# luisdamiano/sparseRGPs

Hardware: AMD Instinct MI355X
Metric: sparse-GP objective+gradient evals/sec at n=1e6, m=1024, d=8 (higher is better)
Workload: dtype f64; 1 GPU; C3: Titsias VI ELBO + gradient, n=1000000, m=1024, d=8, ard, P=10, knots fixed; n=1000000, m=1024, d=8, kernel=ard, parallelism=single

## Files before the change

include/sgp_diag.h:

```cpp
#ifndef SGP_DIAG_H
#define SGP_DIAG_H

#include <stdint.h>

#ifdef __cplusplus
extern "C" {
#endif

int sgp_diag_gj_pair(int device, int64_t m, const double* A, const double* B, double beta,
                     int per_step, double* invA, double* invS, double* logdet);

int sgp_diag_store_bw(int device, int64_t bytes, int reps, int pattern, double* gbs);

int sgp_diag_syrk_plan(int64_t n, int64_t m, int* plan, int* workgroups, double* t_balanced,
                       double* t_packed);

#ifdef __cplusplus
}
#endif
#endif
```

sparsergps_amd/_lib.py:

```python
from __future__ import annotations

import ctypes as C
import os
import threading

from ._build import LIB, VARIANT_ROOT, HipccMissing, build

_lock = threading.Lock()
_lib = None

c_double_p = C.POINTER(C.c_double)
c_int_p = C.POINTER(C.c_int)

SGP_OK, SGP_EINVAL, SGP_ENOTPD, SGP_EHIP, SGP_ENOMEM = 0, 1, 2, 3, 4
KERNELS = {"sqexp": 0, "ard": 1, "exp": 2}
SGP_FLAG_R_DET = 1
SGP_FLAG_OBJ_ONLY = 2
SGP_PRED_VI, SGP_PRED_LAPLACE, SGP_PRED_FULL, SGP_PRED_LAPLACE_FULL = 0, 1, 2, 3
SGP_EXPO_ROWS = 0.0
FAMILIES = {"poisson": 0, "bernoulli": 1}

PROTOTYPES = {
    "sgp_last_error": (C.c_char_p, []),
    "sgp_abi_version": (C.c_int, []),
# ... 24 lines not shown
                                C.c_double, C.c_uint, c_double_p, c_double_p]),
    "sgp_vi_red1_count": (C.c_int64, [C.c_int64]),
    "sgp_vi_red1_packed_count": (C.c_int64, [C.c_int64]),
    "sgp_ctx_set_packed_reduction": (C.c_int, [C.c_void_p, C.c_int]),
    "sgp_vi_red2_count": (C.c_int64, [C.c_int, C.c_int]),
    "sgp_vi_phase1": (C.c_int, [C.c_void_p, C.c_int, c_double_p, c_double_p, C.c_int64, C.c_int64,
                                C.c_double, C.c_void_p]),
    "sgp_vi_phase2": (C.c_int, [C.c_void_p, C.c_void_p, C.c_int64, C.c_uint, C.c_void_p]),
    "sgp_vi_finish": (C.c_int, [C.c_void_p, C.c_void_p, c_double_p, c_double_p]),
    "sgp_fitc_red1_count": (C.c_int64, [C.c_int64]),
    "sgp_fitc_red2_count": (C.c_int64, [C.c_int, C.c_int, C.c_int64]),
    "sgp_fitc_phase1": (C.c_int, [C.c_void_p, C.c_int, c_double_p, c_double_p, C.c_int64, C.c_int64,
                                  C.c_double, C.c_void_p]),
    "sgp_fitc_phase2": (C.c_int, [C.c_void_p, C.c_void_p, C.c_int64, C.c_uint, C.c_void_p]),
    "sgp_fitc_finish": (C.c_int, [C.c_void_p, C.c_void_p, c_double_p, c_double_p]),
    "sgp_lap_set_f": (C.c_int, [C.c_void_p, c_double_p, C.c_double]),
    "sgp_lap_set_expo": (C.c_int, [C.c_void_p, c_double_p, C.c_double]),
    "sgp_lap_set_family": (C.c_int, [C.c_void_p, C.c_int]),
    "sgp_diag_gj_pair": (C.c_int, [C.c_int, C.c_int64, c_double_p, c_double_p, C.c_double, C.c_int,
                                   c_double_p, c_double_p, c_double_p]),
    "sgp_diag_store_bw": (C.c_int, [C.c_int, C.c_int64, C.c_int, C.c_int, c_double_p]),
    "sgp_diag_syrk_plan": (C.c_int, [C.c_int64, C.c_int64, c_int_p, c_int_p, c_double_p,
                                     c_double_p]),
    "sgp_lap_get_f": (C.c_int, [C.c_void_p, c_double_p]),
    "sgp_lap_get_grad_psi": (C.c_int, [C.c_void_p, c_double_p]),
    "sgp_lap_objective_values": (C.c_int, [C.c_void_p, c_double_p, C.c_int, c_int_p]),
    "sgp_eval_laplace": (C.c_int, [C.c_void_p, C.c_int, c_double_p, c_double_p, C.c_int64,
                                   C.c_int64, C.c_double, C.c_double, C.c_double, C.c_int,
                                   c_double_p, c_double_p, c_int_p]),
    "sgp_lap_red_count": (C.c_int64, [C.c_int, C.c_int, C.c_int64]),
    "sgp_lap_begin": (C.c_int, [C.c_void_p, C.c_int, c_double_p, c_double_p, C.c_int64, C.c_int64,
                                C.c_double, C.c_double, C.c_double, C.c_int, C.c_uint,
                                C.c_void_p, C.POINTER(C.c_int64)]),
    "sgp_lap_step": (C.c_int, [C.c_void_p, C.c_void_p, C.c_void_p, C.POINTER(C.c_int64), c_int_p,
                               c_double_p, c_double_p, c_int_p]),
    "sgp_lap_nr": (C.c_int, [C.c_void_p, C.c_int, c_double_p, c_double_p, C.c_int64, C.c_int64,
                             C.c_double, C.c_double, C.c_double, C.c_int, c_double_p, c_int_p]),
    "sgp_eval_full": (C.c_int, [C.c_void_p, C.c_int, c_double_p, C.c_double, C.c_uint,
                                c_double_p, c_double_p]),
    "sgp_eval_full_laplace": (C.c_int, [C.c_void_p, C.c_int, c_double_p, C.c_double, C.c_double,
                                        C.c_double, C.c_int, C.c_uint, c_double_p, c_double_p,
                                        c_int_p]),
    "sgp_full_laplace_state": (C.c_int, [C.c_void_p, c_double_p, c_double_p]),
    "sgp_posterior_u": (C.c_int, [C.c_void_p, c_double_p, c_double_p, c_double_p]),
    "sgp_predict": (C.c_int, [C.c_int, C.c_int, c_double_p, C.c_double, C.c_int, C.c_int, c_double_p,
                              C.c_int64, C.c_int64, c_double_p, c_double_p, c_double_p, C.c_int64,
# ... 90 lines not shown
```

sparsergps_amd/csrc/capi.hip:

```cpp
#include <math.h>

#include <cmath>
#include <stdarg.h>
#include <stdio.h>
#include <stdlib.h>
#include <string.h>
#include <time.h>

#include <algorithm>
#include <string>
#include <vector>

#include "../../include/sgp.h"
#include "../../include/sgp_diag.h"
#include "sgp_internal.h"

#ifdef SGP_HOST_PROBE
extern "C" __attribute__((visibility("default"))) double sgp_probe_t[4] = {0.0, 0.0, 0.0, 0.0};
#endif
#include "sgp_probe.h"
#include "sgp_multi.h"

namespace {

// ... 170 lines not shown
  double* r = nullptr;
  double* K = nullptr;
  double* alpha = nullptr;
  double* zinv = nullptr;
  double* omega = nullptr;
  double* pvec = nullptr;
  double* rowq = nullptr;
  double* red2f = nullptr;
  double* U = nullptr;
  double *K22 = nullptr, *K22inv = nullptr, *Bm = nullptr, *Binv = nullptr, *Pm = nullptr;
  double *Xt = nullptr, *T1 = nullptr, *M3 = nullptr;
  double *Xt22 = nullptr, *T22 = nullptr;
  unsigned* gjs = nullptr;
  double *dinv = nullptr, *dinv22 = nullptr, *logd22 = nullptr, *logdB = nullptr;
  double *uvec = nullptr, *cdiag = nullptr;
  int* status = nullptr;
  double *red1 = nullptr, *red2 = nullptr;
  double *slab_syrk = nullptr, *slab_con = nullptr, *slab_small = nullptr, *sc = nullptr;
  double* sk_ws = nullptr;
  unsigned* sk_flags = nullptr;
  unsigned sk_epoch = 0;
  int sk_slots = 0;
  double* tslab = nullptr;
  double *tq = nullptr, *tp = nullptr;
  int tstore_state = 0;
  int64_t slab_syrk_cap = 0, slab_con_cap = 0, slab_small_cap = 0;
  KernParams kp;
  int64_t m = 0, mp = 0, n_global = 0;
  double delta = 0.0;
  unsigned flags = 0;
  bool knot_on = false;
  double *knot_slab = nullptr, *knot_part = nullptr, *knot_kmm = nullptr;
  std::vector<double> knot_raw;
  std::vector<double> hU;
  double* pin = nullptr;
  hipEvent_t ev_pin = nullptr;
  bool knots_valid = false;
  int64_t knots_mp = 0;
  uint64_t* khash = nullptr;
  int* kidx = nullptr;
  uint8_t* cflag = nullptr;
  int64_t knots_gen = 0;
  int64_t cflag_gen = -1;
  std::vector<double> xmin, xmax;
  int phase = 0;
  int last_mode = 0;
// ... 193 lines not shown
    } else {
      (void)hipGetLastError();
      if (c->tq) (void)hipFree(c->tq);
      if (c->tp) (void)hipFree(c->tp);
      c->tq = c->tp = nullptr;
      c->tstore_state = -1;
    }
  }
  return c->tstore_state == 1;
}

static bool fuse_tt(sgp_ctx* c) { return c->kp.d <= 8 && tstore_ready(c); }

void ctx_free(sgp_ctx* c) {
  void* ptrs[] = {c->X,      c->r,     c->K,      c->alpha,   c->zinv,  c->U,    c->K22,
                  c->K22inv, c->Bm,    c->Binv,   c->Pm,      c->Xt,    c->T1,   c->M3,
                  c->dinv,   c->logd22, c->logdB, c->uvec,    c->cdiag, c->status, c->red1,
                  c->red2,   c->slab_syrk, c->slab_con, c->slab_small, c->slab_aux, c->sc,
                  c->sk_ws,  c->sk_flags,
                  c->Xt22,   c->T22,    c->dinv22, c->omega, c->pvec, c->rowq, c->red2f,
                  c->y,      c->mu,     c->lv,     c->lm,    c->lslab, c->lred[0], c->lred[1],
                  c->Cprev,  c->lapAZ,  c->lapAB,  c->laprv,  c->fl,
                  c->knot_slab, c->knot_part, c->knot_kmm, c->tslab, c->tq, c->tp,
                  c->rr_dev, c->Sfull, c->gjs, c->mmpart, c->rsync};
  for (void* p : ptrs)
    if (p) hipFree(p);
  if (c->khash) hipFree(c->khash);
  if (c->kidx) hipFree(c->kidx);
  if (c->cflag) hipFree(c->cflag);
  if (c->ev_knots) hipEventDestroy(c->ev_knots);
  if (c->ev_pin) hipEventDestroy(c->ev_pin);
  if (c->pin) hipHostFree(c->pin);
  if (c->ev_k22) hipEventDestroy(c->ev_k22);
  if (c->ev_k22m) hipEventDestroy(c->ev_k22m);
  if (c->ev_s) hipEventDestroy(c->ev_s);
  if (c->ev_m3) hipEventDestroy(c->ev_m3);
  if (c->ev_bm) hipEventDestroy(c->ev_bm);
  if (c->ev_lo) hipEventDestroy(c->ev_lo);
  if (c->ev_t) hipEventDestroy(c->ev_t);
  if (c->aux && !c->borrowed_streams) hipStreamDestroy(c->aux);
  if (c->aux_lo && !c->borrowed_streams) hipStreamDestroy(c->aux_lo);
  for (hipEvent_t e : c->pool) hipEventDestroy(e);
  if (c->own && !c->borrowed_streams) hipStreamDestroy(c->own);
}

hipError_t upload_rows(double* dst, const double* src, int64_t n, int64_t n_pad) {
  std::vector<double> h((size_t)n_pad, 0.0);
// ... 337 lines not shown
  if (con_sk_enabled()) {
    int cus = 0;
    if (!st && hipDeviceGetAttribute(&cus, hipDeviceAttributeMultiprocessorCount, device) ==
                   hipSuccess && cus > 0)
      c->sk_slots = 2 * cus;
    if (c->sk_slots > 0) {
      st = st ? st : dalloc(&c->sk_ws, sgp_con_sk_doubles(c->sk_slots));
      st = st ? st : dalloc(&c->sk_flags, c->sk_slots + 1);
      if (!st && hipMemset(c->sk_flags, 0, sizeof(unsigned) * (c->sk_slots + 1)) != hipSuccess) {
        set_err("hipMemset of the contraction hand-over flags failed");
        st = SGP_EHIP;
      }
    }
  }
  c->slab_small_cap = std::max<int64_t>(SLAB_SMALL, mp * (SGP_MAXD + 2));
  st = st ? st : dalloc(&c->slab_small, c->slab_small_cap);
  st = st ? st : dalloc(&c->slab_aux, c->slab_small_cap);
  st = st ? st : dalloc(&c->rr_dev, 1);
  st = st ? st : dalloc(&c->mmpart, 3 * mp);
  st = st ? st : dalloc(&c->sc, SC_N);
  st = st ? st : dalloc(&c->y, np_);
  st = st ? st : dalloc(&c->mu, np_);
  st = st ? st : dalloc(&c->tslab, (np_ / 64) * mp);
  st = st ? st : dalloc(&c->khash, mp);
  st = st ? st : dalloc(&c->kidx, mp);
  st = st ? st : dalloc(&c->cflag, np_);
  if (!st && (hipHostMalloc(reinterpret_cast<void**>(&c->pin),
                            sizeof(double) * (mp * d + m_max + (m_max + 1) / 2 + 8 + RB_N),
                            hipHostMallocDefault) != hipSuccess ||
              hipEventCreateWithFlags(&c->ev_pin, hipEventDisableTiming) != hipSuccess)) {
    set_err("pinned staging allocation failed");
    st = SGP_ENOMEM;
  }
  if (st) {
    ctx_free(c);
    delete c;
    return st;
  }
  c->xmin.assign((size_t)d, 0.0);
  c->xmax.assign((size_t)d, 0.0);
  for (int q = 0; q < d; ++q) {
    double lo = X[q * ldx], hi = X[q * ldx];
    for (int64_t i = 1; i < n; ++i) {
      const double v = X[i + q * ldx];
      lo = v < lo ? v : lo;
      hi = v > hi ? v : hi;
// ... 358 lines not shown
    Scope t(c, "build_knm");
    if (SGP_VI_BUILD_NO_T)
      HIPCHK(launch_build_knm(kp, c->X, c->n_pad, c->n, c->n_pad, c->U, mpv, m, mpv, c->K,
                              c->stream, false));
    else
      HIPCHK(launch_build_knm_t(kp, c->X, c->n_pad, c->n, c->n_pad, c->U, mpv, m, mpv, c->K,
                                c->r, c->tslab, &t_rows, c->stream, false));
  }
  st = k22_sync(c);
  if (st) return st;
  {
    Scope t(c, "syrk");
    HIPCHK(launch_syrk_aug(c->K, c->n_pad, mpv, c->r, nullptr, c->slab_syrk, c->slab_syrk_cap,
                           red1, c->stream, 1, nullptr, 0));
  }
  HIPCHK(hipMemsetAsync(c->status, 0, sizeof(int) * 4, c->aux));
  HIPCHK(hipMemsetAsync(c->sc, 0, sizeof(double) * SC_N, c->aux));
  st = k22_build(c, kp.tau2);
  if (st) return st;
  const int64_t toff = vi_red1_toff(c, mpv);
  if (small_syrk && c->fused_vi) {
    c->t_deferred = true;
    c->t_rows_def = t_rows;
  } else if (small_syrk) {
    HIPCHK(launch_knot_reduce(c->tslab, t_rows, mpv, 1, c->T1, c->mp_max * c->mp_max,
                              red1 + toff, false, c->stream));
  } else {
    HIPCHK(hipStreamWaitEvent(c->aux_lo, c->ev_knots, 0));
    HIPCHK(hipMemsetAsync(red1, 0, sizeof(double) * (toff + mpv + 8), c->aux_lo));
    HIPCHK(launch_knot_reduce(c->tslab, t_rows, mpv, 1, c->T1, c->mp_max * c->mp_max,
                              red1 + toff, false, c->aux_lo));
    HIPCHK(hipStreamWaitEvent(c->aux_lo, c->ev_k22m, 0));
    HIPCHK(hipEventRecord(c->ev_lo, c->aux_lo));
    HIPCHK(hipStreamWaitEvent(c->stream, c->ev_lo, 0));
  }
  {
    Scope t(c, "syrk_reduce");
    HIPCHK(launch_syrk_aug(c->K, c->n_pad, mpv, c->r, nullptr, c->slab_syrk, c->slab_syrk_cap,
                           red1, c->stream, 2, nullptr, 0, c->rr_dev, c->pack_red1, false,
                           c->rsync));
  }
  const bool k22_after_syrk = (double)c->n_pad * (double)mpv * (double)mpv > 3e10;
  st = k22_factor(c, k22_after_syrk);
  if (st) return st;
  c->phase = 1;
  return SGP_OK;
}

static int k22_factor_launches(sgp_ctx* c, hipStream_t s) {
  const int64_t mp = c->mp;
  HIPCHK(dense_spd_inverse(c->K22inv, mp, c->Xt22, c->dinv22, c->logd22, c->status,
                           c->gjs + SGP_GJ_SYNC_WORDS, s));
  HIPCHK(launch_sum_and_diag(c->logd22, mp / SGP_DB, c->sc + SC_LD22, c->K22inv, mp, mp,
                             c->cdiag, s));
  return SGP_OK;
}

static int k22_sync(sgp_ctx* c) {
// ... 103 lines not shown
    HIPCHK(hipEventRecord(c->ev_bm, c->stream));
  }
  {
    HIPCHK(hipStreamWaitEvent(c->aux_lo, c->ev_bm, 0));
    HIPCHK(launch_vi_mm_scalars(t, c->uvec, c->mmpart, mp, red1 + toff + mp, c->sc + SC_TU,
                                c->sc + SC_TRBS, c->sc + SC_RR, c->aux_lo));
    HIPCHK(launch_sum_small(c->logdB, mp / SGP_DB, c->sc + SC_LDB, c->aux_lo));
    Scope tm(c, "contract_kmm", c->aux_lo);
    int nb = 0;
    HIPCHK(launch_contract_kmm(kp, c->U, c->mp, c->m, mp, c->uvec, c->K22inv, c->Binv, c->M3,
                               -0.5, 0.5, -1.0 / (2.0 * kp.tau2), nullptr, nullptr, 0.0,
                               c->slab_aux, c->slab_small_cap, &nb, c->aux_lo));
    HIPCHK(launch_colsum(c->slab_aux, nb, kp.P, c->sc + SC_G22, c->aux_lo));
  }
  int st2 = SGP_OK;
  {
    Scope tm(c, "contract_knm");
    ConArgs ca;
    ca.r = c->r;
    ca.invz = 1.0 / z;
    ca.uvec = c->uvec;
    ca.cdiag = c->cdiag;
    ca.vi_fold = true;
    st2 = contract_pass(c, c->Pm, ca, red2, red2 + sgp_vi_red2_count(kp.kernel, kp.d), false);
  }
  if (!st2)
    HIPCHK(launch_vi_fold_cols(kp, S, c->Pm, t, c->uvec, c->U, c->mp, c->m, mp, 1.0 / z,
                               red1 + toff + mp, c->mmpart + mp, !c->knot_on, c->sc + SC_ESIG,
                               c->sc + SC_EL, c->sc + SC_ATA, c->aux_lo));
  HIPCHK(hipEventRecord(c->ev_m3, c->aux_lo));
  if (st2) return st2;
  HIPCHK(hipStreamWaitEvent(c->stream, c->ev_m3, 0));
  c->phase = 2;
  return SGP_OK;
}

int sgp_vi_finish(sgp_ctx* c, const double* red2, double* obj, double* grad) {
  MULTI_REFUSE(c, "sgp_vi_finish");
  const bool obj_only = c && (c->flags & SGP_FLAG_OBJ_ONLY);
  if (!c || !red2 || !obj || (!grad && !obj_only)) {
    set_err("invalid arguments");
    return SGP_EINVAL;
  }
  if (c->phase != 2) { set_err("sgp_vi_finish called before sgp_vi_phase2"); return SGP_EINVAL; }
  {
    const hipError_t e = hipSetDevice(c->device);
// ... 1721 lines not shown
    if (err == hipSuccess) err = hipEventSynchronize(e1);
    float ms = 0.0f;
    if (err == hipSuccess) err = hipEventElapsedTime(&ms, e0, e1);
    if (err == hipSuccess && r > 0 && ms > 0.0f) best = std::max(best, (double)used / (ms * 1e6));
  }
  (void)hipEventDestroy(e0);
  (void)hipEventDestroy(e1);
  HIPCHK(err);
  *gbs = best;
  return SGP_OK;
}

int sgp_diag_syrk_plan(int64_t n, int64_t m, int* plan, int* workgroups, double* t_balanced,
                       double* t_packed) {
  if (n < 1 || m < 1 || !plan || !workgroups || !t_balanced || !t_packed) {
    set_err("invalid sgp_diag_syrk_plan arguments");
    return SGP_EINVAL;
  }
  syrk_plan_info(round_up(n, SGP_TILE), round_up(m, SGP_TILE), plan, workgroups, t_balanced,
                 t_packed);
  return SGP_OK;
}

}
```

sparsergps_amd/csrc/k_mfma.hip:

```cpp
#include <algorithm>
#include <vector>

#include "sgp_internal.h"
#include "sgp_probe.h"
#include "sgp_syrk_plan.h"

namespace {

constexpr int T128 = 128;
constexpr int BK = 16;
constexpr int SB = 144;
constexpr int SA = 17;
constexpr int SYRK_RGRP = 16;

__device__ __forceinline__ double wave_sum(double v) {
#pragma unroll
  for (int o = 32; o > 0; o >>= 1) v += __shfl_xor(v, o, 64);
  return v;
}

__device__ __forceinline__ int64_t xcd_remap(int64_t orig, int64_t nwg) {
  return sgp_plan::xcd_remap(orig, nwg);
}

// ... 1107 lines not shown

template <int DT, int EPI, bool V2, bool KNOT, bool FROM_T, bool KU, bool T2, int SKM,
          bool VIF = false>
__device__ __forceinline__ void con_tile(
    const KernParams& kp, const double* __restrict__ K, const double* __restrict__ M,
    const double* __restrict__ X, int64_t ldx, int64_t n, int64_t n_pad,
    const double* __restrict__ U, int64_t ldu, int64_t m, int64_t mp, const ConArgs& ca,
    double* __restrict__ slab, int nrec, double* __restrict__ rowq, int64_t ti, int64_t tj,
    int64_t wgid, int kb, int ke, double* lds, double (*red)[SGP_MAXD + 5], double (*s_uk)[BK],
    const ConSK& sk, int part, int tid_in) {
  const double* __restrict__ r = ca.r;
  const double* __restrict__ uvec = ca.uvec;
  const double* __restrict__ cdiag = ca.cdiag;
  constexpr int A_SZ = CON_A_SZ, B_SZ = CON_B_SZ;
  const int64_t ntj = mp / T128;
  const int64_t nwg = (n_pad / T128) * ntj;
  const int64_t i0 = ti * T128, j0 = tj * T128;

  const int tid = tid_in, lane = tid & 63, wv = tid >> 6;
  const int wr = wv >> 1, wc = wv & 1;
  const bool with_u = KU && (uvec != nullptr) && (ca.alpha_in == nullptr);
  constexpr bool with_v = V2;
  constexpr bool NOCS = VIF && !KNOT;
  constexpr bool RING = con_ring<FROM_T, KU, SKM, VIF>();

  d4 acc[4][4];
#pragma unroll
  for (int a = 0; a < 4; ++a)
#pragma unroll
    for (int b = 0; b < 4; ++b) acc[a][b] = d4{0.0, 0.0, 0.0, 0.0};

  const int arow = tid >> 1, acol = (tid & 1) * 8;
  const double2* gA = reinterpret_cast<const double2*>(K + (i0 + arow) * mp + acol);
  const int bk = tid >> 4, bc = tid & 15;
  const double2* gB = reinterpret_cast<const double2*>(M + (int64_t)bk * mp + j0) + bc;
  const int64_t bstep = BK * mp / 2;
  double2 va0, va1, va2, va3, vb0, vb1, vb2, vb3;
  double ku = 0.0, vuk = 0.0;
  const double* __restrict__ uk_src = with_u ? uvec : M;

#define CON_GLOAD(step)                                                          \
  {                                                                              \
    const int64_t oa_ = (int64_t)(step) * (BK / 2), ob_ = (int64_t)(step) * bstep; \
    va0 = gA[oa_]; va1 = gA[oa_ + 1]; va2 = gA[oa_ + 2]; va3 = gA[oa_ + 3];      \
    vb0 = gB[ob_]; vb1 = gB[ob_ + 16]; vb2 = gB[ob_ + 32]; vb3 = gB[ob_ + 48];   \
    if constexpr (KU) vuk = uk_src[(int64_t)(step) * BK + (tid & (BK - 1))];     \
// ... 183 lines not shown
  double* s_u = s_rs + T128;
  double* s_cd = s_u + T128;
  double* s_beta = s_cd + T128;
  double* s_v = s_beta + T128;
  double* s_xs = s_v + T128;
  double* s_us = s_xs + T128 * 16;
  double* s_rs2 = lds + 8320;
  static_assert(8320 + T128 <= 2 * (A_SZ + B_SZ), "s_rs2 fits the LDS image");
  ku += __shfl_xor(ku, 1, 64);
  double a2 = 0.0;
  if ((tid & 1) == 0) {
    const int64_t i = i0 + arow;
    double iz, al;
    if constexpr (VIF) {
      iz = ca.invz;
      al = r[i] * iz;
    } else {
      iz = ca.invz_vec ? ca.invz_vec[i] : ca.invz;
      al = ca.alpha_in ? ca.alpha_in[i]
                       : (with_u ? (r[i] - ku) * iz : 0.0);
    }
    const bool iv = i < n;
    s_alpha[arow] = iv ? al : 0.0;
    s_rs[arow] = iv ? (ca.rs_vec ? ca.rs * ca.rs_vec[i] : ca.rs) : 0.0;
    if constexpr (T2) s_rs2[arow] = iv ? (ca.rs_vec2 ? ca.rs2 * ca.rs_vec2[i] : ca.rs2) : 0.0;
    s_beta[arow] = (with_v && iv) ? ca.beta_in[i] : 0.0;
    if constexpr (!VIF) {
      if (tj == 0) {
        if (ca.count_a2 && i < n) a2 = al * al;
        if (ca.alpha_out) ca.alpha_out[i] = al;
      }
    }
  }
  const double* Kt = K + i0 * mp + j0;

  if constexpr (EPI == EPI_ROWQUAD) {
    if (ca.tstore != nullptr) {
#pragma unroll
      for (int fm = 0; fm < 4; ++fm)
#pragma unroll
        for (int fn = 0; fn < 4; ++fn)
#pragma unroll
          for (int q = 0; q < 4; ++q)
            ca.tstore[(i0 + wr * 64 + fm * 16 + (lane >> 4) + 4 * q) * mp + j0 + wc * 64 +
                      fn * 16 + (lane & 15)] = acc[fm][fn][q];
    }
    __syncthreads();
    double* s_q = s_cd;
#pragma unroll
// ... 11 lines not shown
        double v = 0.0;
#pragma unroll
        for (int fn = 0; fn < 4; ++fn)
          v = fma(kv[q][fn], acc[fm][fn][q], v);
        v += __shfl_xor(v, 1, 64);
        v += __shfl_xor(v, 2, 64);
        v += __shfl_xor(v, 4, 64);
        v += __shfl_xor(v, 8, 64);
        if ((lane & 15) == 0) s_q[wc * T128 + row] = v;
      }
    }
    __syncthreads();
    if (tid < T128) rowq[tj * n_pad + i0 + tid] = s_q[tid] + s_q[T128 + tid];
    return;
  } else {
    const int d = kp.d;
    constexpr int sus = 9;
    const bool ard = (kp.kernel == 1);
    const double rl2s = kp.rl2[0];
    const int L = kp.L;
    for (int e = tid; e < T128; e += 256) {
      const int64_t j = j0 + e;
      s_u[e] = (uvec && j < m) ? uvec[j] : 0.0;
      s_v[e] = (with_v && j < m) ? ca.vvec[j] : 0.0;
      s_cd[e] = (cdiag && j < m) ? cdiag[j] : 0.0;
    }
    double e_sig = 0.0;
    double e_sq = 0.0;
    double* s_kn;
    static_assert(DT % 8 == 0, "coordinates are processed in chunks of 8");
    constexpr int NCH = DT / 8;
    {
      constexpr int KST = 136;
      const double* const kq0 = K + (i0 + (wv >> 1) * 64 + 4 * (wv & 1)) * mp + j0 + 2 * lane;
      double* kst = s_us + ((T128 * sus + 1) & ~1);
#define CON_XSTAGE(ch_)                                                                  \
      _Pragma("unroll") for (int e = tid; e < T128 * 8; e += 256) {                      \
        const int rr = e % T128, c = e / T128, cg = 8 * (ch_) + c;                       \
        const int64_t i = i0 + rr, j = j0 + rr;                                          \
        double xv = 0.0;                                                                 \
        if (cg < d) {                                                                    \
          const double sc = ard ? kp.rl[cg] : 1.0;                                       \
          xv = (i < n) ? X[i + cg * ldx] * sc : 0.0;                                     \
          s_us[rr * sus + c] = (j < m) ? U[j + cg * ldu] * sc : 0.0;                     \
        }                                                                                \
        s_xs[rr * 16 + c] = xv;                                                          \
        s_xs[rr * 16 + 8 + c] = xv * xv;                                                 \
      }
#ifdef SGP_CON_PROBE_NO_KDMA
#define CON_KHALF(s_)
#else
#define CON_KHALF(s_)                                                                    \
      _Pragma("unroll") for (int q_ = 0; q_ < 4; ++q_) {                                 \
        const int rho_ = wv * 4 + q_;                                                    \
        __builtin_amdgcn_global_load_lds(                                                \
            (const __attribute__((address_space(1))) void*)(                             \
                kq0 + (int64_t)(((s_) >> 1) * 16 + ((s_) & 1) * 8 + q_) * mp),          \
            (__attribute__((address_space(3))) void*)(kst + ((s_) & 1) * 16 * KST + rho_ * KST), \
            16, 0, 0);                                                                   \
// ... 29 lines not shown
      }
      {
#pragma unroll
        for (int hs = 0; hs < 8; ++hs) {
          const int fm = hs >> 1, h = hs & 1;
          if (hs > 0) {
            __builtin_amdgcn_s_waitcnt(0);
            __syncthreads();
            if (hs < 7) { CON_KHALF(hs + 1); }
          }
          double t2c[2][4];
          if constexpr (T2) {
#pragma unroll
            for (int r2 = 0; r2 < 2; ++r2)
#pragma unroll
              for (int fn = 0; fn < 4; ++fn) t2c[r2][fn] = t2n[r2][fn];
            if (hs < 7) { CON_T2LOAD(hs + 1); }
          }
          const double* kb = kst + h * 16 * KST;
          double xb[2];
#pragma unroll
          for (int r2 = 0; r2 < 2; ++r2)
            xb[r2] = s_xs[(wr * 64 + fm * 16 + 4 * (2 * h + r2) + (lane >> 4)) * 16 + (lane & 15)];
#pragma unroll
          for (int fn = 0; fn < 4; ++fn) {
            const int col = wc * 64 + fn * 16 + (lane & 15);
            double kv[2];
#pragma unroll
            for (int r2 = 0; r2 < 2; ++r2) kv[r2] = kb[(wr * 8 + (lane >> 4) + 4 * r2) * KST + col];
#pragma unroll
            for (int r2 = 0; r2 < 2; ++r2) {
              const int q = 2 * h + r2;
              const int row = wr * 64 + fm * 16 + (lane >> 4) + 4 * q;
              double G = s_rs[row] * acc[fm][fn][q];
              if constexpr (T2) G = fma(s_rs2[row], t2c[r2][fn], G);
              if constexpr (V2) G = fma(s_beta[row], vcol[fn], G);
              G = fma(s_alpha[row], ucol[fn], G);
              double w = G * kv[r2];
              if constexpr ((V2 && KNOT) || FROM_T) w = (j0 + col < m && i0 + row < n) ? w : 0.0;
              if constexpr (!NOCS) Cc[fn] += w;
              acc[fm][fn][q] = w;
            }
          }
#pragma unroll
          for (int r2 = 0; r2 < 2; ++r2)
#pragma unroll
            for (int fn = 0; fn < 4; ++fn)
#ifndef SGP_CON_PROBE_NO_EPI_MFMA
              P[fn] = __builtin_amdgcn_mfma_f64_16x16x4f64(acc[fm][fn][2 * h + r2], xb[r2], P[fn],
                                                           0, 0, 0);
#else
              P[fn][r2] = fma(acc[fm][fn][2 * h + r2], xb[r2], P[fn][r2]);
#endif
          if (hs == 1) SGP_PROBE_CON_STAMP(3);
        }
        __syncthreads();
      }
#undef CON_KHALF
#undef CON_T2LOAD
      SGP_PROBE_CON_STAMP(5);
      const int cp = lane & 15, cc = cp & 7;
#pragma unroll
      for (int ch = 0; ch < NCH; ++ch) {
        if (8 * ch >= d) break;
        if (ch > 0) {
          __syncthreads();
          CON_XSTAGE(ch);
          __syncthreads();
#pragma unroll
          for (int fn = 0; fn < 4; ++fn) P[fn] = d4{0.0, 0.0, 0.0, 0.0};
#pragma unroll
          for (int fm = 0; fm < 4; ++fm) {
            double xb[4];
#pragma unroll
            for (int r4 = 0; r4 < 4; ++r4)
              xb[r4] = s_xs[(wr * 64 + fm * 16 + 4 * r4 + (lane >> 4)) * 16 + (lane & 15)];
#pragma unroll
            for (int r4 = 0; r4 < 4; ++r4)
#pragma unroll
              for (int fn = 0; fn < 4; ++fn)
                P[fn] = __builtin_amdgcn_mfma_f64_16x16x4f64(acc[fm][fn][r4], xb[r4], P[fn], 0,
                                                             0, 0);
          }
        }
        const bool cok = 8 * ch + cc < d;
        double E = 0.0;
#pragma unroll
        for (int fn = 0; fn < 4; ++fn) {
          if constexpr (NOCS) {
#pragma unroll
            for (int q = 0; q < 4; ++q) {
              const int jl = wc * 64 + fn * 16 + (lane >> 4) + 4 * q;
              const double u = cok ? s_us[jl * sus + cc] : 0.0;
              const double pv = P[fn][q];
              E += (cp >= 8) ? pv : -2.0 * (u * pv);
            }
          } else {
          double C = Cc[fn];
          C += __shfl_xor(C, 16, 64);
          C += __shfl_xor(C, 32, 64);
          if (ch == 0 && (lane >> 4) == 0) e_sig += C;
#pragma unroll
          for (int q = 0; q < 4; ++q) {
            const int jl = wc * 64 + fn * 16 + (lane >> 4) + 4 * q;
            const double Cq = __shfl(C, (lane >> 4) + 4 * q, 64);
            const double u = cok ? s_us[jl * sus + cc] : 0.0;
            const double pv = P[fn][q];
            E += (cp >= 8) ? pv : u * fma(u, Cq, -2.0 * pv);
            if constexpr (KNOT) {
              if (cp < 8) s_kn[(wr * T128 + jl) * 8 + cc] = pv - u * Cq;
            }
          }
          }
        }
        E += __shfl_xor(E, 8, 64);
        E += __shfl_xor(E, 16, 64);
        E += __shfl_xor(E, 32, 64);
        if (ard) {
          if (lane < 8 && 8 * ch + lane < d) red[wv][1 + 8 * ch + lane] = E;
        } else {
          double t = E;
          t += __shfl_xor(t, 1, 64);
          t += __shfl_xor(t, 2, 64);
          t += __shfl_xor(t, 4, 64);
          e_sq += t;
        }
        if constexpr (KNOT) {
          __syncthreads();
          for (int e = tid; e < T128 * 8; e += 256) {
            const int col = e >> 3, c = e & 7, cg = 8 * ch + c;
            if (cg < d)
              ca.knot_slab[(ti * mp + j0 + col) * d + cg] =
                  s_kn[col * 8 + c] + s_kn[(T128 + col) * 8 + c];
          }
        }
      }
#undef CON_XSTAGE
    }

    SGP_PROBE_CON_STAMP(6);
    double v = 0.0;
    if constexpr (!NOCS) v = wave_sum(e_sig);
    if (lane == 0) red[wv][0] = v;
    if (!ard && lane == 0) red[wv][1] = e_sq * rl2s;
    v = 0.0;
    if constexpr (!VIF) v = wave_sum(a2);
    if (lane == 0) {
      red[wv][1 + L] = 0.0;
      red[wv][2 + L] = 0.0;
      red[wv][3 + L] = 0.0;
      red[wv][4 + L] = v;
    }
    __syncthreads();
    if (tid < nrec)
      slab[tid * nwg + wgid] = red[0][tid] + red[1][tid] + red[2][tid] + red[3][tid];
    SGP_PROBE_CON_STAMP(2);
  }
  if constexpr (SGP_CON_EPI_PRIO > 0) __builtin_amdgcn_s_setprio(0);
}

// ... 813 lines not shown
    hipLaunchKernelGGL((k_contract<DT, EPI_GRAD, false, false, true, true, T2>), g, b, 0, s, kp,
                       K, M, X, ldx, n, n_pad, U, ldu, m, mp, ca, slab, nrec, (double*)nullptr);
}

template <int DT>
static void launch_con_from_t(bool v2, bool kn, const KernParams& kp, const double* K,
                              const double* M, const double* X, int64_t ldx, int64_t n,
                              int64_t n_pad, const double* U, int64_t ldu, int64_t m, int64_t mp,
                              const ConArgs& ca, double* slab, int nrec, int64_t nwg,
                              hipStream_t s) {
  if constexpr (DT == 8) {
    if (ca.tin2 != nullptr) {
      launch_con_from_t2<DT, true>(v2, kn, kp, K, M, X, ldx, n, n_pad, U, ldu, m, mp, ca, slab,
                                   nrec, nwg, s);
      return;
    }
  }
    launch_con_from_t2<DT, false>(v2, kn, kp, K, M, X, ldx, n, n_pad, U, ldu, m, mp, ca, slab,
                                  nrec, nwg, s);
}

int64_t sgp_con_sk_doubles(int slots) { return (int64_t)(slots + 1) * CON_SK_SLOT; }

hipError_t launch_contract_args(const KernParams& kp, const double* K, const double* M,
                                const double* X, int64_t ldx, int64_t n, int64_t n_pad,
                                const double* U, int64_t ldu, int64_t m, int64_t mp,
                                const ConArgs& ca, double* slab, int64_t* nrec_out,
                                int64_t* nwg_out, hipStream_t s) {
  const int64_t nwg = (n_pad / T128) * (mp / T128);
  const int nrec = kp.L + 5;
  *nrec_out = nrec;
  *nwg_out = nwg;
  if ((ca.tin2 != nullptr) != (ca.M2 != nullptr) || (ca.tin2 && (!ca.tin || kp.d > 8)))
    return hipErrorInvalidValue;
  if (ca.vi_fold && (ca.tin || ca.beta_in || ca.alpha_in || ca.invz_vec || !ca.uvec || !ca.r))
    return hipErrorInvalidValue;
  if (ca.tin != nullptr) {
    if (ca.uvec != nullptr && ca.alpha_in == nullptr) return hipErrorInvalidValue;
    const bool v2 = ca.beta_in != nullptr, kn = ca.knot_slab != nullptr;
    if (kp.d <= 8) launch_con_from_t<8>(v2, kn, kp, K, M, X, ldx, n, n_pad, U, ldu, m, mp, ca, slab,
                                        nrec, nwg, s);
    else launch_con_from_t<SGP_MAXD>(v2, kn, kp, K, M, X, ldx, n, n_pad, U, ldu, m, mp, ca, slab,
                                     nrec, nwg, s);
    return hipGetLastError();
  }
  if (ca.knot_slab != nullptr) {
    const bool v2 = ca.beta_in != nullptr;
    if (kp.d <= 8) launch_con_grad<8, true>(v2, kp, K, M, X, ldx, n, n_pad, U, ldu, m, mp, ca,
                                            slab, nrec, nwg, s);
    else launch_con_grad<SGP_MAXD, true>(v2, kp, K, M, X, ldx, n, n_pad, U, ldu, m, mp, ca, slab,
                                         nrec, nwg, s);
  } else {
    const bool v2 = ca.beta_in != nullptr;
    if (kp.d <= 8) launch_con_grad<8>(v2, kp, K, M, X, ldx, n, n_pad, U, ldu, m, mp, ca, slab,
                                      nrec, nwg, s);
    else launch_con_grad<SGP_MAXD>(v2, kp, K, M, X, ldx, n, n_pad, U, ldu, m, mp, ca, slab, nrec,
                                   nwg, s);
  }
// ... 73 lines not shown
```

sparsergps_amd/csrc/sgp_internal.h:

```cpp
#pragma once
#include <hip/hip_runtime.h>
#include <stdint.h>

#define SGP_MAXD 32
#define SGP_TILE 128
#define SGP_DB 64
#define SGP_GJ_SYNC_WORDS (128 + 2 * 64 * 64)

typedef double d4 __attribute__((ext_vector_type(4)));

__device__ __forceinline__ double sgp_exp_nonpos(double x) {
  constexpr double c2 = 1.0 / 2, c3 = 1.0 / 6, c4 = 1.0 / 24, c5 = 1.0 / 120, c6 = 1.0 / 720,
                   c7 = 1.0 / 5040, c8 = 1.0 / 40320, c9 = 1.0 / 362880, c10 = 1.0 / 3628800,
                   c11 = 1.0 / 39916800, c12 = 1.0 / 479001600, c13 = 1.0 / 6227020800.0;
  const double k = __builtin_rint(x * 1.4426950408889634074);
  double r = __builtin_fma(-k, 6.93147180369123816490e-01, x);
  r = __builtin_fma(-k, 1.90821492927058770002e-10, r);
  double p = c13;
  p = __builtin_fma(p, r, c12);
  p = __builtin_fma(p, r, c11);
  p = __builtin_fma(p, r, c10);
  p = __builtin_fma(p, r, c9);
  p = __builtin_fma(p, r, c8);
  p = __builtin_fma(p, r, c7);
// ... 93 lines not shown
                           bool packed = false,
                           bool w_nonneg = false,
                           unsigned* rsync = nullptr);
#define SGP_SYRK_RSYNC_WORDS 4096
int64_t syrk_packed_doubles(int64_t mp);
hipError_t launch_unpack_lower64(const double* packed, int64_t mp, double* S, hipStream_t s);
int64_t syrk_slab_doubles(int64_t n_pad, int64_t mp);
void syrk_plan_info(int64_t n_pad, int64_t mp, int* plan, int* nwg, double* t_bal, double* t_pack);
bool syrk_use_s256(int64_t mp, bool with_t);
struct ConArgs {
  const double* r = nullptr;
  double invz = 0.0;
  const double* invz_vec = nullptr;
  const double* uvec = nullptr;
  const double* alpha_in = nullptr;
  const double* beta_in = nullptr;
  const double* vvec = nullptr;
  const double* rs_vec = nullptr;
  double rs = 1.0;
  const double* cdiag = nullptr;
  int count_a2 = 0;
  double* alpha_out = nullptr;
  bool vi_fold = false;
  double* knot_slab = nullptr;
  double* tstore = nullptr;
  const double* tin = nullptr;
  const double* tin2 = nullptr;
  const double* M2 = nullptr;
  const double* rs_vec2 = nullptr;
  double rs2 = 0.0;
  double* sk_ws = nullptr;
  unsigned* sk_flags = nullptr;
  unsigned sk_epoch = 0;
  int sk_slots = 0;
  int* sk_status = nullptr;
  int sk_dp = -1;
};
int64_t sgp_con_sk_doubles(int slots);
hipError_t launch_contract_args(const KernParams& kp, const double* K, const double* M,
                                const double* X, int64_t ldx, int64_t n, int64_t n_pad,
                                const double* U, int64_t ldu, int64_t m, int64_t mp,
                                const ConArgs& ca, double* slab, int64_t* nrec_out,
                                int64_t* nwg_out, hipStream_t s);
hipError_t launch_contract_knm(const KernParams& kp, const double* K, const double* M,
                               const double* X, int64_t ldx, int64_t n, int64_t n_pad,
                               const double* U, int64_t ldu, int64_t m, int64_t mp,
                               const double* r, double invz, const double* invz_vec,
                               const double* uvec, const double* rs_vec, double rs,
                               const double* coinc_diag, int count_a2, double* slab,
                               int64_t* nrec_out, int64_t* nwg_out, hipStream_t s);
hipError_t launch_rowquad_knm(const KernParams& kp, const double* K, const double* M, int64_t n,
                              int64_t n_pad, int64_t m, int64_t mp, const double* r,
                              double invz, const double* invz_vec, const double* uvec,
                              double* alpha_out, double* rowq_slab, double* out,
                              hipStream_t s, double* tstore = nullptr);
hipError_t launch_gemm64(bool transA, bool transB, bool lower_only, int64_t M, int64_t N,
                         int64_t K, double alpha, const double* A, int64_t lda,
                         const double* B, int64_t ldb, double beta, double* C, int64_t ldc,
                         hipStream_t s);

// ... 139 lines not shown
```

Measured before the change: 22.01 evals/s.

## Precompute scaled X/U images and stage them via direct LDS loads in VI contraction

Adds a kernel on the low-priority aux stream that writes lengthscale-scaled X rows (with their squares) and scaled knot coordinates into per-channel images. The VI-fold contraction then stages them with global_load_lds and plain copies instead of recomputing the scaling in every tile. A LEAN path also drops the rs/beta/v/cdiag shared loads and fmas that are always trivial in VI mode. The cost is an extra n_pad*16-double buffer, a write-and-read pass over it, and a full waitcnt before each channel stage. A diagnostic accessor for the images is also added.

Measured after the change: 22.02 evals/s (median of 2 runs). No clear change (+0.1%).

```diff
diff --git a/include/sgp_diag.h b/include/sgp_diag.h
--- a/include/sgp_diag.h
+++ b/include/sgp_diag.h
@@ -15,6 +15,10 @@
 int sgp_diag_syrk_plan(int64_t n, int64_t m, int* plan, int* workgroups, double* t_balanced,
                        double* t_packed);
 
+struct sgp_ctx;
+int sgp_diag_con_images(struct sgp_ctx* ctx, double* xb, int64_t xb_len, double* us,
+                        int64_t us_len);
+
 #ifdef __cplusplus
 }
 #endif
diff --git a/sparsergps_amd/_lib.py b/sparsergps_amd/_lib.py
--- a/sparsergps_amd/_lib.py
+++ b/sparsergps_amd/_lib.py
@@ -70,6 +70,7 @@
     "sgp_diag_store_bw": (C.c_int, [C.c_int, C.c_int64, C.c_int, C.c_int, c_double_p]),
     "sgp_diag_syrk_plan": (C.c_int, [C.c_int64, C.c_int64, c_int_p, c_int_p, c_double_p,
                                      c_double_p]),
+    "sgp_diag_con_images": (C.c_int, [C.c_void_p, c_double_p, C.c_int64, c_double_p, C.c_int64]),
     "sgp_lap_get_f": (C.c_int, [C.c_void_p, c_double_p]),
     "sgp_lap_get_grad_psi": (C.c_int, [C.c_void_p, c_double_p]),
     "sgp_lap_objective_values": (C.c_int, [C.c_void_p, c_double_p, C.c_int, c_int_p]),
diff --git a/sparsergps_amd/csrc/capi.hip b/sparsergps_amd/csrc/capi.hip
--- a/sparsergps_amd/csrc/capi.hip
+++ b/sparsergps_amd/csrc/capi.hip
@@ -216,6 +216,8 @@
   unsigned sk_epoch = 0;
   int sk_slots = 0;
   double* tslab = nullptr;
+  double *con_xb = nullptr, *con_us = nullptr;
+  int64_t con_img_mp = 0;
   double *tq = nullptr, *tp = nullptr;
   int tstore_state = 0;
   int64_t slab_syrk_cap = 0, slab_con_cap = 0, slab_small_cap = 0;
@@ -455,7 +457,7 @@
                   c->y,      c->mu,     c->lv,     c->lm,    c->lslab, c->lred[0], c->lred[1],
                   c->Cprev,  c->lapAZ,  c->lapAB,  c->laprv,  c->fl,
                   c->knot_slab, c->knot_part, c->knot_kmm, c->tslab, c->tq, c->tp,
-                  c->rr_dev, c->Sfull, c->gjs, c->mmpart, c->rsync};
+                  c->rr_dev, c->Sfull, c->gjs, c->mmpart, c->rsync, c->con_xb, c->con_us};
   for (void* p : ptrs)
     if (p) hipFree(p);
   if (c->khash) hipFree(c->khash);
@@ -839,6 +841,8 @@
   st = st ? st : dalloc(&c->y, np_);
   st = st ? st : dalloc(&c->mu, np_);
   st = st ? st : dalloc(&c->tslab, (np_ / 64) * mp);
+  st = st ? st : dalloc(&c->con_xb, sgp_con_xb_doubles(np_, d));
+  st = st ? st : dalloc(&c->con_us, sgp_con_us_doubles(mp, d));
   st = st ? st : dalloc(&c->khash, mp);
   st = st ? st : dalloc(&c->kidx, mp);
   st = st ? st : dalloc(&c->cflag, np_);
@@ -1243,18 +1247,29 @@
   if (small_syrk && c->fused_vi) {
     c->t_deferred = true;
     c->t_rows_def = t_rows;
+    HIPCHK(hipStreamWaitEvent(c->aux_lo, c->ev_knots, 0));
+    HIPCHK(launch_con_images(kp, c->X, c->n_pad, c->n, c->n_pad, c->U, mpv, m, mpv, c->con_xb,
+                             c->con_us, c->aux_lo));
   } else if (small_syrk) {
     HIPCHK(launch_knot_reduce(c->tslab, t_rows, mpv, 1, c->T1, c->mp_max * c->mp_max,
                               red1 + toff, false, c->stream));
+    HIPCHK(hipStreamWaitEvent(c->aux_lo, c->ev_knots, 0));
+    HIPCHK(launch_con_images(kp, c->X, c->n_pad, c->n, c->n_pad, c->U, mpv, m, mpv, c->con_xb,
+                             c->con_us, c->aux_lo));
+    HIPCHK(hipEventRecord(c->ev_lo, c->aux_lo));
+    HIPCHK(hipStreamWaitEvent(c->stream, c->ev_lo, 0));
   } else {
     HIPCHK(hipStreamWaitEvent(c->aux_lo, c->ev_knots, 0));
     HIPCHK(hipMemsetAsync(red1, 0, sizeof(double) * (toff + mpv + 8), c->aux_lo));
     HIPCHK(launch_knot_reduce(c->tslab, t_rows, mpv, 1, c->T1, c->mp_max * c->mp_max,
                               red1 + toff, false, c->aux_lo));
+    HIPCHK(launch_con_images(kp, c->X, c->n_pad, c->n, c->n_pad, c->U, mpv, m, mpv, c->con_xb,
+                             c->con_us, c->aux_lo));
     HIPCHK(hipStreamWaitEvent(c->aux_lo, c->ev_k22m, 0));
     HIPCHK(hipEventRecord(c->ev_lo, c->aux_lo));
     HIPCHK(hipStreamWaitEvent(c->stream, c->ev_lo, 0));
   }
+  c->con_img_mp = mpv;
   {
     Scope t(c, "syrk_reduce");
     HIPCHK(launch_syrk_aug(c->K, c->n_pad, mpv, c->r, nullptr, c->slab_syrk, c->slab_syrk_cap,
@@ -1404,6 +1419,8 @@
     ca.uvec = c->uvec;
     ca.cdiag = c->cdiag;
     ca.vi_fold = true;
+    ca.xb = c->con_xb;
+    ca.us = c->con_us;
     st2 = contract_pass(c, c->Pm, ca, red2, red2 + sgp_vi_red2_count(kp.kernel, kp.d), false);
   }
   if (!st2)
@@ -3171,4 +3188,26 @@
   return SGP_OK;
 }
 
-}
+int sgp_diag_con_images(sgp_ctx* c, double* xb, int64_t xb_len, double* us, int64_t us_len) {
+  MULTI_REFUSE(c, "sgp_diag_con_images");
+  if (!c || !xb || !us) { set_err("invalid sgp_diag_con_images arguments"); return SGP_EINVAL; }
+  if (c->con_img_mp == 0) {
+    set_err("sgp_diag_con_images: no VI evaluation has run on this context");
+    return SGP_EINVAL;
+  }
+  const int64_t nx = sgp_con_xb_doubles(c->n_pad, c->d), nu = sgp_con_us_doubles(c->con_img_mp, c->d);
+  if (xb_len != nx || us_len != nu) {
+    set_err("sgp_diag_con_images: xb_len = %lld (expected %lld), us_len = %lld (expected %lld)",
+            (long long)xb_len, (long long)nx, (long long)us_len, (long long)nu);
+    return SGP_EINVAL;
+  }
+  HIPCHK(hipSetDevice(c->device));
+  HIPCHK(hipStreamSynchronize(c->stream));
+  HIPCHK(hipStreamSynchronize(c->aux));
+  HIPCHK(hipStreamSynchronize(c->aux_lo));
+  HIPCHK(hipMemcpy(xb, c->con_xb, sizeof(double) * nx, hipMemcpyDeviceToHost));
+  HIPCHK(hipMemcpy(us, c->con_us, sizeof(double) * nu, hipMemcpyDeviceToHost));
+  return SGP_OK;
+}
+
+}
diff --git a/sparsergps_amd/csrc/k_mfma.hip b/sparsergps_amd/csrc/k_mfma.hip
--- a/sparsergps_amd/csrc/k_mfma.hip
+++ b/sparsergps_amd/csrc/k_mfma.hip
@@ -1153,6 +1153,7 @@
   const bool with_u = KU && (uvec != nullptr) && (ca.alpha_in == nullptr);
   constexpr bool with_v = V2;
   constexpr bool NOCS = VIF && !KNOT;
+  constexpr bool LEAN = VIF && !(KNOT && DT > 8);
   constexpr bool RING = con_ring<FROM_T, KU, SKM, VIF>();
 
   d4 acc[4][4];
@@ -1382,9 +1383,10 @@
     }
     const bool iv = i < n;
     s_alpha[arow] = iv ? al : 0.0;
-    s_rs[arow] = iv ? (ca.rs_vec ? ca.rs * ca.rs_vec[i] : ca.rs) : 0.0;
+    if constexpr (!LEAN)
+      s_rs[arow] = iv ? (ca.rs_vec ? ca.rs * ca.rs_vec[i] : ca.rs) : 0.0;
     if constexpr (T2) s_rs2[arow] = iv ? (ca.rs_vec2 ? ca.rs2 * ca.rs_vec2[i] : ca.rs2) : 0.0;
-    s_beta[arow] = (with_v && iv) ? ca.beta_in[i] : 0.0;
+    if constexpr (!LEAN) s_beta[arow] = (with_v && iv) ? ca.beta_in[i] : 0.0;
     if constexpr (!VIF) {
       if (tj == 0) {
         if (ca.count_a2 && i < n) a2 = al * al;
@@ -1442,8 +1444,10 @@
     for (int e = tid; e < T128; e += 256) {
       const int64_t j = j0 + e;
       s_u[e] = (uvec && j < m) ? uvec[j] : 0.0;
-      s_v[e] = (with_v && j < m) ? ca.vvec[j] : 0.0;
-      s_cd[e] = (cdiag && j < m) ? cdiag[j] : 0.0;
+      if constexpr (!LEAN) {
+        s_v[e] = (with_v && j < m) ? ca.vvec[j] : 0.0;
+        s_cd[e] = (cdiag && j < m) ? cdiag[j] : 0.0;
+      }
     }
     double e_sig = 0.0;
     double e_sq = 0.0;
@@ -1454,7 +1458,28 @@
       constexpr int KST = 136;
       const double* const kq0 = K + (i0 + (wv >> 1) * 64 + 4 * (wv & 1)) * mp + j0 + 2 * lane;
       double* kst = s_us + ((T128 * sus + 1) & ~1);
+#define CON_XIMG(ch_)                                                                    \
+      {                                                                                  \
+        const double* xsrc_ = ca.xb + ((int64_t)(ch_) * n_pad + i0) * 16 + 2 * lane;     \
+        _Pragma("unroll") for (int q_ = 0; q_ < 4; ++q_)                                 \
+          __builtin_amdgcn_global_load_lds(                                              \
+              (const __attribute__((address_space(1))) void*)(xsrc_ + (wv * 4 + q_) * 128), \
+              (__attribute__((address_space(3))) void*)(s_xs + (wv * 4 + q_) * 128), 16, 0, \
+              0);                                                                        \
+        const double2* usrc_ =                                                           \
+            reinterpret_cast<const double2*>(ca.us + ((int64_t)(ch_) * mp + j0) * 8);    \
+        _Pragma("unroll") for (int k_ = 0; k_ < 2; ++k_) {                               \
+          const int e_ = tid + 256 * k_;           \
+          const double2 u2_ = usrc_[e_];                                                 \
+          double* pu_ = &s_us[(e_ >> 2) * sus + 2 * (e_ & 3)];                           \
+          pu_[0] = u2_.x;                                                                \
+          pu_[1] = u2_.y;                                                                \
+        }                                                                                \
+      }
 #define CON_XSTAGE(ch_)                                                                  \
+      if constexpr (LEAN) CON_XIMG(ch_)                                                  \
+      else { CON_XCALC(ch_) }
+#define CON_XCALC(ch_)                                                                   \
       _Pragma("unroll") for (int e = tid; e < T128 * 8; e += 256) {                      \
         const int rr = e % T128, c = e / T128, cg = 8 * (ch_) + c;                       \
         const int64_t i = i0 + rr, j = j0 + rr;                                          \
@@ -1530,6 +1555,12 @@
 #pragma unroll
           for (int r2 = 0; r2 < 2; ++r2)
             xb[r2] = s_xs[(wr * 64 + fm * 16 + 4 * (2 * h + r2) + (lane >> 4)) * 16 + (lane & 15)];
+          double arow2[2];
+          if constexpr (LEAN) {
+#pragma unroll
+            for (int r2 = 0; r2 < 2; ++r2)
+              arow2[r2] = s_alpha[wr * 64 + fm * 16 + (lane >> 4) + 4 * (2 * h + r2)];
+          }
 #pragma unroll
           for (int fn = 0; fn < 4; ++fn) {
             const int col = wc * 64 + fn * 16 + (lane & 15);
@@ -1540,10 +1571,15 @@
             for (int r2 = 0; r2 < 2; ++r2) {
               const int q = 2 * h + r2;
               const int row = wr * 64 + fm * 16 + (lane >> 4) + 4 * q;
-              double G = s_rs[row] * acc[fm][fn][q];
-              if constexpr (T2) G = fma(s_rs2[row], t2c[r2][fn], G);
-              if constexpr (V2) G = fma(s_beta[row], vcol[fn], G);
-              G = fma(s_alpha[row], ucol[fn], G);
+              double G;
+              if constexpr (LEAN) {
+                G = fma(arow2[r2], ucol[fn], acc[fm][fn][q]);
+              } else {
+                G = s_rs[row] * acc[fm][fn][q];
+                if constexpr (T2) G = fma(s_rs2[row], t2c[r2][fn], G);
+                if constexpr (V2) G = fma(s_beta[row], vcol[fn], G);
+                G = fma(s_alpha[row], ucol[fn], G);
+              }
               double w = G * kv[r2];
               if constexpr ((V2 && KNOT) || FROM_T) w = (j0 + col < m && i0 + row < n) ? w : 0.0;
               if constexpr (!NOCS) Cc[fn] += w;
@@ -1574,6 +1610,7 @@
         if (ch > 0) {
           __syncthreads();
           CON_XSTAGE(ch);
+          if constexpr (LEAN) __builtin_amdgcn_s_waitcnt(0);
           __syncthreads();
 #pragma unroll
           for (int fn = 0; fn < 4; ++fn) P[fn] = d4{0.0, 0.0, 0.0, 0.0};
@@ -1599,7 +1636,7 @@
 #pragma unroll
             for (int q = 0; q < 4; ++q) {
               const int jl = wc * 64 + fn * 16 + (lane >> 4) + 4 * q;
-              const double u = cok ? s_us[jl * sus + cc] : 0.0;
+              const double u = (LEAN || cok) ? s_us[jl * sus + cc] : 0.0;
               const double pv = P[fn][q];
               E += (cp >= 8) ? pv : -2.0 * (u * pv);
             }
@@ -1612,7 +1649,7 @@
           for (int q = 0; q < 4; ++q) {
             const int jl = wc * 64 + fn * 16 + (lane >> 4) + 4 * q;
             const double Cq = __shfl(C, (lane >> 4) + 4 * q, 64);
-            const double u = cok ? s_us[jl * sus + cc] : 0.0;
+            const double u = (LEAN || cok) ? s_us[jl * sus + cc] : 0.0;
             const double pv = P[fn][q];
             E += (cp >= 8) ? pv : u * fma(u, Cq, -2.0 * pv);
             if constexpr (KNOT) {
@@ -1644,6 +1681,8 @@
         }
       }
 #undef CON_XSTAGE
+#undef CON_XCALC
+#undef CON_XIMG
     }
 
     SGP_PROBE_CON_STAMP(6);
@@ -2503,6 +2542,55 @@
 
 int64_t sgp_con_sk_doubles(int slots) { return (int64_t)(slots + 1) * CON_SK_SLOT; }
 
+__global__ void __launch_bounds__(256)
+k_con_images(KernParams kp, const double* __restrict__ X, int64_t ldx, int64_t n, int64_t n_pad,
+             const double* __restrict__ U, int64_t ldu, int64_t m, int64_t mp, int nbx,
+             double* __restrict__ xb, double* __restrict__ us) {
+  const int d = kp.d, ch = (int)blockIdx.y;
+  const bool ard = (kp.kernel == 1);
+  const bool rows = (int)blockIdx.x < nbx;
+  const int64_t e = (int64_t)(rows ? blockIdx.x : blockIdx.x - nbx) * 256 + threadIdx.x;
+  if (e >= (rows ? n_pad : mp)) return;
+  const double* __restrict__ src = rows ? X : U;
+  const int64_t ld = rows ? ldx : ldu;
+  const bool in = e < (rows ? n : m);
+  double v[8];
+#pragma unroll
+  for (int c = 0; c < 8; ++c) {
+    const int cg = 8 * ch + c;
+    double xv = 0.0;
+    if (cg < d) {
+      const double sc = ard ? kp.rl[cg] : 1.0;
+      xv = in ? src[e + cg * ld] * sc : 0.0;
+    }
+    v[c] = xv;
+  }
+  if (rows) {
+    double2* o = reinterpret_cast<double2*>(xb + ((int64_t)ch * n_pad + e) * 16);
+#pragma unroll
+    for (int c = 0; c < 4; ++c) {
+      o[c] = double2{v[2 * c], v[2 * c + 1]};
+      o[4 + c] = double2{v[2 * c] * v[2 * c], v[2 * c + 1] * v[2 * c + 1]};
+    }
+  } else {
+    double2* o = reinterpret_cast<double2*>(us + ((int64_t)ch * mp + e) * 8);
+#pragma unroll
+    for (int c = 0; c < 4; ++c) o[c] = double2{v[2 * c], v[2 * c + 1]};
+  }
+}
+
+int64_t sgp_con_xb_doubles(int64_t n_pad, int d) { return (int64_t)((d + 7) / 8) * n_pad * 16; }
+int64_t sgp_con_us_doubles(int64_t mp, int d) { return (int64_t)((d + 7) / 8) * mp * 8; }
+
+hipError_t launch_con_images(const KernParams& kp, const double* X, int64_t ldx, int64_t n,
+                             int64_t n_pad, const double* U, int64_t ldu, int64_t m, int64_t mp,
+                             double* xb, double* us, hipStream_t s) {
+  const int nbx = (int)((n_pad + 255) / 256), nbu = (int)((mp + 255) / 256);
+  hipLaunchKernelGGL(k_con_images, dim3((unsigned)(nbx + nbu), (unsigned)((kp.d + 7) / 8)),
+                     dim3(256), 0, s, kp, X, ldx, n, n_pad, U, ldu, m, mp, nbx, xb, us);
+  return hipGetLastError();
+}
+
 hipError_t launch_contract_args(const KernParams& kp, const double* K, const double* M,
                                 const double* X, int64_t ldx, int64_t n, int64_t n_pad,
                                 const double* U, int64_t ldu, int64_t m, int64_t mp,
@@ -2514,7 +2602,8 @@
   *nwg_out = nwg;
   if ((ca.tin2 != nullptr) != (ca.M2 != nullptr) || (ca.tin2 && (!ca.tin || kp.d > 8)))
     return hipErrorInvalidValue;
-  if (ca.vi_fold && (ca.tin || ca.beta_in || ca.alpha_in || ca.invz_vec || !ca.uvec || !ca.r))
+  if (ca.vi_fold && (ca.tin || ca.beta_in || ca.alpha_in || ca.invz_vec || !ca.uvec || !ca.r ||
+                     ca.rs_vec || ca.rs != 1.0 || !ca.xb || !ca.us))
     return hipErrorInvalidValue;
   if (ca.tin != nullptr) {
     if (ca.uvec != nullptr && ca.alpha_in == nullptr) return hipErrorInvalidValue;
diff --git a/sparsergps_amd/csrc/sgp_internal.h b/sparsergps_amd/csrc/sgp_internal.h
--- a/sparsergps_amd/csrc/sgp_internal.h
+++ b/sparsergps_amd/csrc/sgp_internal.h
@@ -139,6 +139,8 @@
   int count_a2 = 0;
   double* alpha_out = nullptr;
   bool vi_fold = false;
+  const double* xb = nullptr;
+  const double* us = nullptr;
   double* knot_slab = nullptr;
   double* tstore = nullptr;
   const double* tin = nullptr;
@@ -153,6 +155,11 @@
   int* sk_status = nullptr;
   int sk_dp = -1;
 };
+int64_t sgp_con_xb_doubles(int64_t n_pad, int d);
+int64_t sgp_con_us_doubles(int64_t mp, int d);
+hipError_t launch_con_images(const KernParams& kp, const double* X, int64_t ldx, int64_t n,
+                             int64_t n_pad, const double* U, int64_t ldu, int64_t m, int64_t mp,
+                             double* xb, double* us, hipStream_t s);
 int64_t sgp_con_sk_doubles(int slots);
 hipError_t launch_contract_args(const KernParams& kp, const double* K, const double* M,
                                 const double* X, int64_t ldx, int64_t n, int64_t n_pad,
```
